# dremovd/PPO

Measured on AMD Instinct MI355X. Metric: env-steps/sec (Pong-shaped synthetic, 256 envs/GPU), higher is better.
Workload: dtype f32

## Files before the change

### ppo_amd/csrc/stack_fused.hip

```cpp
#include <cstdlib>
#include <type_traits>

#include "common.h"
#include "conv_stage.h"
#include "mfma.h"

#ifndef PPO_TAIL_SPLIT
#define PPO_TAIL_SPLIT 2
#endif

namespace ppo {
namespace {

constexpr int kScrPitchS = 20;

struct StackTailArgs {
    const float *in;
    const float *w[4];
    const float *bias[4];
    const float *mask[4];
    float *save[4];
    int n_images;
};

template <int C, int H, int W, int MT, int NW, int NSPLIT>
struct StackCfg {
    static constexpr int ROWS = H + 2;
    static constexpr int G = 4;
    static constexpr int PLANE_RAW = ROWS * W + 2 * G;
    static constexpr int PLANE = PLANE_RAW + ((16 - PLANE_RAW % 32) + 32) % 32;
    static constexpr int NT = C / 16;
    static constexpr int NTL = NT / NSPLIT;
    static constexpr int WAVES = NW * NSPLIT;
    static constexpr int KS = 9 * (C / 4);
    static constexpr int NPIX = H * W;
    static constexpr int MTILES = (NPIX + 15) / 16;
    static constexpr int LDS_MAP = C * PLANE;
    static constexpr size_t LDS_BYTES = (size_t)2 * LDS_MAP * 4;
    static_assert(C % 16 == 0, "channel tiles of 16");
    static_assert(MTILES == MT * NW, "one group of MT pixel tiles per wave");
    static_assert(NT % NSPLIT == 0, "channel tiles split evenly");
};

template <int C, int H, int W, int MT, int NW, int NSPLIT, bool BACKWARD>
__global__ __launch_bounds__(NW * NSPLIT * 64) void stack_tail_kernel(StackTailArgs a)
{
    using S = StackCfg<C, H, W, MT, NW, NSPLIT>;
    constexpr int NT = S::NTL, KS = S::KS, PLANE = S::PLANE, G = S::G;
    extern __shared__ __align__(16) float smem[];
    const int tid = threadIdx.x, lane = tid & 63, l15 = lane & 15, g = lane >> 4;
    const int wave = (tid >> 6) % NW;
    const int n0 = ((tid >> 6) / NW) * NT;

    zero_lds<2 * S::LDS_MAP, S::WAVES * 64>(smem, tid);
    __syncthreads();

    int pix[MT], lofs[MT];
    float hi_l[MT], hi_r[MT];
#pragma unroll
    for (int m = 0; m < MT; ++m) {
        const int p = (wave * MT + m) * 16 + l15;
        pix[m] = p;
        const int pc = p < S::NPIX ? p : 0;
        lofs[m] = G + pc - 1 + g * PLANE;
        hi_l[m] = (pc % W == 0) ? 0.f : INFINITY;
        hi_r[m] = (pc % W == W - 1) ? 0.f : INFINITY;
    }

    float wa[NT][KS];
    auto load_weights = [&](int layer) {
        const float4 *pw = reinterpret_cast<const float4 *>(a.w[layer]);
#pragma unroll
        for (int s4 = 0; s4 < KS / 4; ++s4)
#pragma unroll
            for (int n = 0; n < NT; ++n) {
                const float4 v = pw[(s4 * S::NT + n0 + n) * 64 + lane];
                wa[n][4 * s4 + 0] = v.x;
                wa[n][4 * s4 + 1] = v.y;
                wa[n][4 * s4 + 2] = v.z;
                wa[n][4 * s4 + 3] = v.w;
            }
    };
    load_weights(0);

    for (int img = blockIdx.x; img < a.n_images; img += gridDim.x) {
        __syncthreads();
        stage_band_chunk_dma<C, H, W, S::ROWS, PLANE, G, S::WAVES>(a.in, img, 0, smem, tid);
        const size_t img_off = (size_t)img * C * H * W;

#pragma unroll 1
        for (int layer = 0; layer < 4; ++layer) {
            float bias_r[NT][4];
#pragma unroll
            for (int n = 0; n < NT; ++n)
#pragma unroll
                for (int r = 0; r < 4; ++r) bias_r[n][r] = BACKWARD ? 0.f : a.bias[layer][(n0 + n) * 16 + g * 4 + r];
            float gate[BACKWARD ? MT : 1][NT][4];
            if constexpr (BACKWARD) {
                const __amdgpu_buffer_rsrc_t mask = buffer_of(a.mask[layer] + img_off);
#pragma unroll
                for (int m = 0; m < MT; ++m)
#pragma unroll
                    for (int n = 0; n < NT; ++n)
#pragma unroll
                        for (int r = 0; r < 4; ++r)
                            gate[m][n][r] = buffer_f32(mask, pix[m] < S::NPIX ? (((n0 + n) * 16 + g * 4 + r) * (H * W) + pix[m]) * 4
                                                                              : kOutside);
            }

            __syncthreads();
            const int odd = layer & 1;
            const int src = odd ? S::LDS_MAP : 0;
            int base[MT];
#pragma unroll
            for (int m = 0; m < MT; ++m) base[m] = lofs[m] + src;

            f32x4 acc[NT][MT];
#pragma unroll
            for (int n = 0; n < NT; ++n)
#pragma unroll
                for (int m = 0; m < MT; ++m) acc[n][m] = f32x4{0.f, 0.f, 0.f, 0.f};

            constexpr int SB = (MT * NT >= 4) ? 2 : 4;
            constexpr int NB = (KS + SB - 1) / SB;
            float raw[2][SB][MT];
            auto load_block = [&](int j, float (&r)[SB][MT]) {
#pragma unroll
                for (int u = 0; u < SB; ++u) {
                    const int s = j * SB + u;
                    if (s < KS) {
                        const int tap = s / (C / 4), cs = s % (C / 4);
                        const int tap_off = (tap / 3) * W + (tap % 3);
#pragma unroll
                        for (int m = 0; m < MT; ++m) r[u][m] = smem[base[m] + cs * 4 * PLANE + tap_off];
                    }
                }
            };
            load_block(0, raw[0]);
#pragma unroll
            for (int j = 0; j < NB; ++j) {
                float bv[SB][MT];
#pragma unroll
                for (int u = 0; u < SB; ++u) {
                    const int s = j * SB + u;
                    if (s < KS) {
                        const int kx = (s / (C / 4)) % 3;
#pragma unroll
                        for (int m = 0; m < MT; ++m) {
                            float x = raw[j & 1][u][m];
                            if (kx != 1) {
                                const float hi = kx == 0 ? hi_l[m] : hi_r[m];
                                x = __builtin_amdgcn_fmed3f(x, BACKWARD ? -hi : 0.f, hi);
                            } else if (!BACKWARD) {
                                x = relu1(x);
                            }
                            bv[u][m] = x;
                        }
                    }
                }
                __builtin_amdgcn_sched_barrier(0);
                if (j + 1 < NB) load_block(j + 1, raw[(j + 1) & 1]);
#pragma unroll
                for (int u = 0; u < SB; ++u) {
                    const int s = j * SB + u;
                    if (s < KS) {
#pragma unroll
                        for (int m = 0; m < MT; ++m)
#pragma unroll
                            for (int n = 0; n < NT; ++n) acc[n][m] = mfma16(wa[n][s], bv[u][m], acc[n][m]);
                    }
                }
                __builtin_amdgcn_sched_barrier(0);
            }

            __builtin_amdgcn_sched_barrier(0);
            load_weights((layer + 1) & 3);
            float *dst = smem + (odd ? 0 : S::LDS_MAP);
            float *save = a.save[layer];
            __builtin_amdgcn_sched_barrier(0);
            float skip[MT][NT][4];
#pragma unroll
            for (int m = 0; m < MT; ++m)
#pragma unroll
                for (int n = 0; n < NT; ++n)
#pragma unroll
                    for (int r = 0; r < 4; ++r)
                        skip[m][n][r] = odd ? smem[((n0 + n) * 16 + g * 4 + r) * PLANE + G + W + (pix[m] < S::NPIX ? pix[m] : 0)] : 0.f;
#pragma unroll
            for (int m = 0; m < MT; ++m) {
                if (pix[m] < S::NPIX) {
#pragma unroll
                    for (int n = 0; n < NT; ++n)
#pragma unroll
                        for (int r = 0; r < 4; ++r) {
                            const int co = (n0 + n) * 16 + g * 4 + r;
                            const int lo = co * PLANE + G + W + pix[m];
                            float val = acc[n][m][r] + bias_r[n][r];
                            if constexpr (BACKWARD) val = gate[m][n][r] > 0.f ? val : 0.f;
                            if (odd) val = val + skip[m][n][r];
                            dst[lo] = val;
                            if (save) save[img_off + (size_t)co * (H * W) + pix[m]] = val;
                        }
                }
            }
        }
    }
}

template <int C, int H, int W, int MT, int NW, int NSPLIT, bool BACKWARD>
int launch_stack_tail(const StackTailArgs &args, hipStream_t st)
{
    using S = StackCfg<C, H, W, MT, NW, NSPLIT>;
    auto kern = stack_tail_kernel<C, H, W, MT, NW, NSPLIT, BACKWARD>;
    static int wg_per_cu = 0;
    if (wg_per_cu == 0) {
        hipError_t e = hipFuncSetAttribute(reinterpret_cast<const void *>(kern), hipFuncAttributeMaxDynamicSharedMemorySize,
                                           (int)S::LDS_BYTES);
        if (e != hipSuccess) return fail(PPO_E_HIP, "stack_tail: hipFuncSetAttribute: %s", hipGetErrorString(e));
        int nb = 0;
        e = hipOccupancyMaxActiveBlocksPerMultiprocessor(&nb, kern, S::WAVES * 64, S::LDS_BYTES);
        if (e != hipSuccess) return fail(PPO_E_HIP, "stack_tail: occupancy query: %s", hipGetErrorString(e));
        wg_per_cu = nb < 1 ? 1 : nb;
    }
    int grid = 256 * wg_per_cu;
    if (grid > args.n_images) grid = args.n_images;
    hipLaunchKernelGGL(kern, dim3(grid), dim3(S::WAVES * 64), S::LDS_BYTES, st, args);
    return check_launch("stack_tail_kernel");
}

template <int C, int H, int W, int TR>
struct ShiftCfg {
    static_assert(C == 16, "one channel tile per wave");
    static constexpr int NW = 16;
    static constexpr int GW = 8;
    static constexpr int G = 4;
    static constexpr int ROWS = H + 6;
    static constexpr int PLANE_RAW = ROWS * W + 2 * G;
    static constexpr int PLANE = PLANE_RAW + ((16 - PLANE_RAW % 32) + 32) % 32;
    static constexpr int KS = 9 * (C / 4);
    static constexpr int NBANDS = (H + TR - 1) / TR;
    static constexpr int NPIX = TR * W;
    static constexpr int MTILES = (NPIX + 15) / 16;
    static constexpr int MT = MTILES / GW;
    static constexpr int LDS_MAP = C * PLANE;
    static constexpr int SCR = MT * 16 * kScrPitchS;
    static constexpr size_t LDS_BYTES = (size_t)(LDS_MAP + GW * SCR) * 4;
    static_assert(H % TR == 0 && MTILES == MT * GW, "whole bands, tiles split evenly over a group's waves");
    static_assert((H * W) % 4 == 0 && NPIX % 4 == 0 && W % 2 == 0, "float4 epilogue on whole quads");
    static_assert(LDS_BYTES <= 160 * 1024, "map + scratch must fit the CU's LDS");
};

template <int C, int H, int W, int TR, bool BACKWARD>
__global__ __launch_bounds__(1024) void stack_shift_kernel(StackTailArgs a)
{
    using S = ShiftCfg<C, H, W, TR>;
    constexpr int KS = S::KS, PLANE = S::PLANE, G = S::G, MT = S::MT, NW = S::NW;
    extern __shared__ __align__(16) float smem[];
    const int tid = threadIdx.x, lane = tid & 63, l15 = lane & 15, g = lane >> 4, wave = tid >> 6;
    const int grp = __builtin_amdgcn_readfirstlane(wave / S::GW), wv = wave % S::GW;
    const int ch = lane >> 2, quad = lane & 3;
    float *scr = smem + S::LDS_MAP + wv * S::SCR;

    int lofs[MT], p4[MT];
    float hi_l[MT], hi_r[MT];
#pragma unroll
    for (int m = 0; m < MT; ++m) {
        const int p = (wv * MT + m) * 16 + l15;
        lofs[m] = G + p - 1 + g * PLANE;
        hi_l[m] = (p % W == 0) ? 0.f : INFINITY;
        hi_r[m] = (p % W == W - 1) ? 0.f : INFINITY;
        p4[m] = (wv * MT + m) * 16 + quad * 4;
    }

    for (int img = blockIdx.x; img < a.n_images; img += gridDim.x) {
        const size_t img_off = (size_t)img * C * H * W;
        __syncthreads();
        for (int i = tid; i < C * 6 * W; i += NW * 64) {
            const int c = i / (6 * W), r = (i / W) % 6, x = i % W;
            smem[c * PLANE + G + (r < 5 ? r : H + 5) * W + x] = 0.f;
        }
        for (int i = tid; i < C * 2 * G; i += NW * 64)
            smem[(i / (2 * G)) * PLANE + ((i % (2 * G)) < G ? (i % G) : G + S::ROWS * W + (i % G))] = 0.f;
        {
            using gptr_t = const __attribute__((address_space(1))) void *;
            using lptr_t = __attribute__((address_space(3))) void *;
            constexpr int N4 = H * W / 4, REQ = (N4 + 63) / 64;
            const int w0 = __builtin_amdgcn_readfirstlane(wave);
            for (int c = w0; c < C; c += NW) {
                const float *g0 = a.in + img_off + (size_t)c * H * W;
                float *l0 = smem + c * PLANE + G + 5 * W;
#pragma unroll
                for (int q = 0; q < REQ; ++q)
                    if (q * 64 + lane < N4)
                        __builtin_amdgcn_global_load_lds((gptr_t)(g0 + (q * 64 + lane) * 4), (lptr_t)(l0 + q * 256), 16, 0, 0);
            }
        }

#pragma unroll 1
        for (int layer = 0; layer < 4; ++layer) {
            float wa[KS];
            const float4 *pw = reinterpret_cast<const float4 *>(a.w[layer]);
#pragma unroll
            for (int s4 = 0; s4 < KS / 4; ++s4) {
                const float4 v = pw[s4 * 64 + lane];
                wa[4 * s4 + 0] = v.x, wa[4 * s4 + 1] = v.y, wa[4 * s4 + 2] = v.z, wa[4 * s4 + 3] = v.w;
            }
            const float bias_c = BACKWARD ? 0.f : a.bias[layer][ch];
            const int odd = layer & 1;
            const float *res = odd ? (layer == 1 ? a.in : a.save[1]) + img_off : nullptr;
            const float *mask = BACKWARD ? a.mask[layer] + img_off : nullptr;
            float *save = a.save[layer] ? a.save[layer] + img_off : nullptr;
            const __amdgpu_buffer_rsrc_t mask_b = buffer_of(mask, mask != nullptr), res_b = buffer_of(res, res != nullptr);
            const int in_row = 5 - layer;

            f32x4 acc[MT];
            float4 gate4[MT], res4[MT];

            __syncthreads();
#pragma unroll 1
            for (int hs = 0; hs <= S::NBANDS; ++hs) {
                if ((hs & 1) == grp) {
                    if (hs < S::NBANDS) {
                        const int y0 = hs * TR;
                        const int chan_off = ch * (H * W) + y0 * W;
#pragma unroll
                        for (int m = 0; m < MT; ++m) {
                            const bool live = p4[m] < S::NPIX;
                            const int off = live ? (chan_off + p4[m]) * 4 : kOutside;
                            if constexpr (BACKWARD) gate4[m] = buffer_f32x4(mask_b, off);
                            res4[m] = buffer_f32x4(res_b, off);
                        }
                        int base[MT];
#pragma unroll
                        for (int m = 0; m < MT; ++m) {
                            base[m] = lofs[m] + (y0 - 1 + in_row) * W;
                            acc[m] = f32x4{0.f, 0.f, 0.f, 0.f};
                        }
                        constexpr int SB = 2;
                        constexpr int NB = (KS + SB - 1) / SB;
                        float raw[2][SB][MT];
                        auto load_block = [&](int j, float (&r)[SB][MT]) {
#pragma unroll
                            for (int u = 0; u < SB; ++u) {
                                const int s = j * SB + u;
                                if (s < KS) {
                                    const int tap = s / (C / 4), cs = s % (C / 4);
                                    const int tap_off = (tap / 3) * W + (tap % 3);
#pragma unroll
                                    for (int m = 0; m < MT; ++m) r[u][m] = smem[base[m] + cs * 4 * PLANE + tap_off];
                                }
                            }
                        };
                        load_block(0, raw[0]);
#pragma unroll
                        for (int j = 0; j < NB; ++j) {
                            float bv[SB][MT];
#pragma unroll
                            for (int u = 0; u < SB; ++u) {
                                const int s = j * SB + u;
                                if (s < KS) {
                                    const int kx = (s / (C / 4)) % 3;
#pragma unroll
                                    for (int m = 0; m < MT; ++m) {
                                        float x = raw[j & 1][u][m];
                                        if (kx != 1) {
                                            const float hi = kx == 0 ? hi_l[m] : hi_r[m];
                                            x = __builtin_amdgcn_fmed3f(x, BACKWARD ? -hi : 0.f, hi);
                                        } else if (!BACKWARD) {
                                            x = relu1(x);
                                        }
                                        bv[u][m] = x;
                                    }
                                }
                            }
                            __builtin_amdgcn_sched_barrier(0);
                            if (j + 1 < NB) load_block(j + 1, raw[(j + 1) & 1]);
#pragma unroll
                            for (int u = 0; u < SB; ++u) {
                                const int s = j * SB + u;
                                if (s < KS) {
#pragma unroll
                                    for (int m = 0; m < MT; ++m) acc[m] = mfma16(wa[s], bv[u][m], acc[m]);
                                }
                            }
                            __builtin_amdgcn_sched_barrier(0);
                        }
                    } else if (layer < 3) {
                        for (int i = tid % (S::GW * 64); i < C * W; i += S::GW * 64)
                            smem[(i / W) * PLANE + G + (H + in_row - 1) * W + i % W] = 0.f;
                    }
                } else if (hs >= 1) {
                    const int y0 = (hs - 1) * TR;
                    const int chan_off = ch * (H * W) + y0 * W;
#pragma unroll
                    for (int m = 0; m < MT; ++m)
#pragma unroll
                        for (int r = 0; r < 4; ++r) scr[(m * 16 + g * 4 + r) * kScrPitchS + l15] = acc[m][r];
                    __builtin_amdgcn_wave_barrier();
                    float *out_row = smem + ch * PLANE + G + (y0 + in_row - 1) * W;
#pragma unroll
                    for (int m = 0; m < MT; ++m) {
                        if (p4[m] >= S::NPIX) continue;
                        const float4 o = *reinterpret_cast<const float4 *>(scr + (m * 16 + ch) * kScrPitchS + quad * 4);
                        const float ov[4] = {o.x, o.y, o.z, o.w};
                        const float gv[4] = {gate4[m].x, gate4[m].y, gate4[m].z, gate4[m].w};
                        const float rv[4] = {res4[m].x, res4[m].y, res4[m].z, res4[m].w};
                        float v[4];
#pragma unroll
                        for (int e = 0; e < 4; ++e) {
                            float val = ov[e] + bias_c;
                            if constexpr (BACKWARD) val = gv[e] > 0.f ? val : 0.f;
                            v[e] = val + rv[e];
                        }
                        if (layer < 3) {
                            *reinterpret_cast<float2 *>(out_row + p4[m]) = make_float2(v[0], v[1]);
                            *reinterpret_cast<float2 *>(out_row + p4[m] + 2) = make_float2(v[2], v[3]);
                        }
                        if (save) *reinterpret_cast<float4 *>(save + chan_off + p4[m]) = make_float4(v[0], v[1], v[2], v[3]);
                    }
                    __builtin_amdgcn_wave_barrier();
                }
                __syncthreads();
            }
        }
    }
}

template <int C, int H, int W, int TR, bool BACKWARD>
int launch_stack_shift(const StackTailArgs &args, hipStream_t st)
{
    using S = ShiftCfg<C, H, W, TR>;
    auto kern = stack_shift_kernel<C, H, W, TR, BACKWARD>;
    static bool attr_set = false;
    if (!attr_set) {
        hipError_t e = hipFuncSetAttribute(reinterpret_cast<const void *>(kern), hipFuncAttributeMaxDynamicSharedMemorySize,
                                           (int)S::LDS_BYTES);
        if (e != hipSuccess) return fail(PPO_E_HIP, "stack_shift: hipFuncSetAttribute: %s", hipGetErrorString(e));
        attr_set = true;
    }
    int grid = 256;
    if (grid > args.n_images) grid = args.n_images;
    hipLaunchKernelGGL(kern, dim3(grid), dim3(S::NW * 64), S::LDS_BYTES, st, args);
    return check_launch("stack_shift_kernel");
}

template <int I, int N, class F>
__device__ __forceinline__ void static_for(F &&f)
{
    if constexpr (I < N) {
        f(std::integral_constant<int, I>{});
        static_for<I + 1, N>(f);
    }
}

struct LaneMap {
    template <int MT>
    struct T {
        int pix[MT], lofs[MT];
        float hi_l[MT], hi_r[MT];
    };
};

template <int H, int W, int PLANE, int G, int MT>
__device__ __forceinline__ void lane_map_init(LaneMap::T<MT> &lm, int pixel_wave, int l15, int g)
{
#pragma unroll
    for (int m = 0; m < MT; ++m) {
        const int p = (pixel_wave * MT + m) * 16 + l15;
        lm.pix[m] = p;
        const int pc = p < H * W ? p : 0;
        lm.lofs[m] = G + pc - 1 + g * PLANE;
        lm.hi_l[m] = (pc % W == 0) ? 0.f : INFINITY;
        lm.hi_r[m] = (pc % W == W - 1) ? 0.f : INFINITY;
    }
}

template <int C, int H, int W, int MT, int NTOT, int NT, bool RELU_IN, bool GATED = false>
__device__ __forceinline__ void resident_conv(float *smem, int src_off, int dst_off, bool residual, const float *wpk,
                                              const float *bias, float *save, const LaneMap::T<MT> &lm, int n0, int lane,
                                              const float *mask = nullptr)
{
    constexpr int ROWS = H + 2, G = 4, PLANE_RAW = ROWS * W + 2 * G;
    constexpr int PLANE = PLANE_RAW + ((16 - PLANE_RAW % 32) + 32) % 32;
    constexpr int KS = 9 * (C / 4);
    const int g = lane >> 4;
    float wa[NT][KS];
    const float4 *pw = reinterpret_cast<const float4 *>(wpk);
#pragma unroll
    for (int s4 = 0; s4 < KS / 4; ++s4)
#pragma unroll
        for (int n = 0; n < NT; ++n) {
            const float4 v = pw[(s4 * NTOT + n0 + n) * 64 + lane];
            wa[n][4 * s4 + 0] = v.x;
            wa[n][4 * s4 + 1] = v.y;
            wa[n][4 * s4 + 2] = v.z;
            wa[n][4 * s4 + 3] = v.w;
        }
    float bias_r[NT][4];
#pragma unroll
    for (int n = 0; n < NT; ++n)
#pragma unroll
        for (int r = 0; r < 4; ++r) bias_r[n][r] = (GATED || !bias) ? 0.f : bias[(n0 + n) * 16 + g * 4 + r];
    float gate[GATED ? MT : 1][NT][4];
    if constexpr (GATED) {
        const __amdgpu_buffer_rsrc_t mask_b = buffer_of(mask);
#pragma unroll
        for (int m = 0; m < MT; ++m)
#pragma unroll
            for (int n = 0; n < NT; ++n)
#pragma unroll
                for (int r = 0; r < 4; ++r)
                    gate[m][n][r] = buffer_f32(mask_b, lm.pix[m] < H * W ? (((n0 + n) * 16 + g * 4 + r) * (H * W) + lm.pix[m]) * 4
                                                                         : kOutside);
    }

    __syncthreads();
    int base[MT];
#pragma unroll
    for (int m = 0; m < MT; ++m) base[m] = lm.lofs[m] + src_off;
    f32x4 acc[NT][MT];
#pragma unroll
    for (int n = 0; n < NT; ++n)
#pragma unroll
        for (int m = 0; m < MT; ++m) acc[n][m] = f32x4{0.f, 0.f, 0.f, 0.f};

    constexpr int SB = (MT * NT >= 4) ? 2 : 4;
    constexpr int NB = (KS + SB - 1) / SB;
    float raw[2][SB][MT];
    auto load_block = [&](int j, float (&r)[SB][MT]) {
#pragma unroll
        for (int u = 0; u < SB; ++u) {
            const int s = j * SB + u;
            if (s < KS) {
                const int tap = s / (C / 4), cs = s % (C / 4);
                const int tap_off = (tap / 3) * W + (tap % 3);
#pragma unroll
                for (int m = 0; m < MT; ++m) r[u][m] = smem[base[m] + cs * 4 * PLANE + tap_off];
            }
        }
    };
    load_block(0, raw[0]);
    static_for<0, NB>([&](auto jc) {
        constexpr int j = decltype(jc)::value;
        float bv[SB][MT];
#pragma unroll
        for (int u = 0; u < SB; ++u) {
            const int s = j * SB + u;
            if (s < KS) {
                const int kx = (s / (C / 4)) % 3;
#pragma unroll
                for (int m = 0; m < MT; ++m) {
                    float x = raw[j & 1][u][m];
                    if (kx != 1) {
                        const float hi = kx == 0 ? lm.hi_l[m] : lm.hi_r[m];
                        x = __builtin_amdgcn_fmed3f(x, RELU_IN ? 0.f : -hi, hi);
                    } else if (RELU_IN) {
                        x = relu1(x);
                    }
                    bv[u][m] = x;
                }
            }
        }
        __builtin_amdgcn_sched_barrier(0);
        if constexpr (j + 1 < NB) load_block(j + 1, raw[(j + 1) & 1]);
#pragma unroll
        for (int u = 0; u < SB; ++u) {
            const int s = j * SB + u;
            if (s < KS) {
#pragma unroll
                for (int m = 0; m < MT; ++m)
#pragma unroll
                    for (int n = 0; n < NT; ++n) acc[n][m] = mfma16(wa[n][s], bv[u][m], acc[n][m]);
            }
        }
        __builtin_amdgcn_sched_barrier(0);
    });
#pragma unroll
    for (int m = 0; m < MT; ++m) {
        if (lm.pix[m] < H * W) {
#pragma unroll
            for (int n = 0; n < NT; ++n)
#pragma unroll
                for (int r = 0; r < 4; ++r) {
                    const int co = (n0 + n) * 16 + g * 4 + r;
                    const int lo = dst_off + co * PLANE + G + W + lm.pix[m];
                    float val = acc[n][m][r] + bias_r[n][r];
                    if constexpr (GATED) val = gate[m][n][r] > 0.f ? val : 0.f;
                    if (residual) val = val + smem[lo];
                    smem[lo] = val;
                    if (save) save[(size_t)co * (H * W) + lm.pix[m]] = val;
                }
        }
    }
}

struct StackFullArgs {
    const float *in;
    const float *w[5];
    const float *bias[5];
    float *pooled;
    uint8_t *argmax;
    float *save[4];
    const float *pre_w[4];
    const float *pre_bias[4];
    float *pre_save[4];
    int has_pre;
    int n_images;
};

template <int C, int HI, int WI, int MTI, int HO, int WO, int MTO, int NW, int NSPLIT>
__global__ __launch_bounds__(NW * NSPLIT * 64) void stack_full_kernel(StackFullArgs a)
{
    using SI = StackCfg<C, HI, WI, MTI, NW, NSPLIT>;
    using SO = StackCfg<C, HO, WO, MTO, NW, NSPLIT>;
    static_assert(HO == (HI + 1) / 2 && WO == (WI + 1) / 2, "3x3 / stride 2 / pad 1 pooling");
    static_assert(2 * SO::LDS_MAP <= SI::LDS_MAP, "the small maps reuse the input map's LDS");
    constexpr int NT = SI::NTL, WAVES = SI::WAVES, THREADS = WAVES * 64;
    constexpr int A_OFF = 0, B_OFF = SI::LDS_MAP, X_OFF = 0, Y_OFF = SO::LDS_MAP;
    extern __shared__ __align__(16) float smem[];
    const int tid = threadIdx.x, lane = tid & 63, l15 = lane & 15, g = lane >> 4;
    const int wave = tid >> 6, pixel_wave = wave % NW, n0 = (wave / NW) * NT;

    LaneMap::T<MTI> lmi;
    LaneMap::T<MTO> lmo;
    lane_map_init<HI, WI, SI::PLANE, SI::G, MTI>(lmi, pixel_wave, l15, g);
    lane_map_init<HO, WO, SO::PLANE, SO::G, MTO>(lmo, pixel_wave, l15, g);

    if (a.has_pre) zero_lds<SI::LDS_MAP, THREADS>(smem + B_OFF, tid);

    for (int img = blockIdx.x; img < a.n_images; img += gridDim.x) {
        __syncthreads();
        zero_lds<SI::LDS_MAP, THREADS>(smem + A_OFF, tid);
        __syncthreads();
        stage_band_chunk_dma<C, HI, WI, SI::ROWS, SI::PLANE, SI::G, WAVES>(a.in, img, 0, smem + A_OFF, tid);
        if (a.has_pre) {
            const size_t big_img = (size_t)img * C * HI * WI;
#pragma unroll 1
            for (int layer = 0; layer < 4; ++layer) {
                const int odd = layer & 1;
                float *save = a.pre_save[layer] ? a.pre_save[layer] + big_img : nullptr;
                resident_conv<C, HI, WI, MTI, SI::NT, NT, true>(smem, odd ? B_OFF : A_OFF, odd ? A_OFF : B_OFF, odd != 0,
                                                                a.pre_w[layer], a.pre_bias[layer], save, lmi, n0, lane);
            }
        }
        resident_conv<C, HI, WI, MTI, SI::NT, NT, false>(smem, A_OFF, B_OFF, false, a.w[0], a.bias[0], nullptr, lmi, n0, lane);
        __syncthreads();
        zero_lds<2 * SO::LDS_MAP, THREADS>(smem + X_OFF, tid);
        __syncthreads();
        {
            constexpr int RPW = 64 / WO;
            const int sub = lane / WO, xo = lane % WO;
            const size_t out_img = (size_t)img * C * HO * WO;
            for (int u0 = wave * RPW; u0 < C * HO; u0 += WAVES * RPW) {
                const int u = u0 + sub;
                const int co = u / HO, yo = u % HO;
                if (sub < RPW && co < C) {
                    const float *src = smem + B_OFF + co * SI::PLANE + SI::G + WI + (2 * yo - 1) * WI + 2 * xo - 1;
                    float best;
                    int best_tap;
                    pool_window_lds<HI % 2 == 0, WI % 2 == 0>(src, WI, yo > 0, 2 * yo + 1 < HI, xo > 0, 2 * xo + 1 < WI, best, best_tap);
                    smem[X_OFF + co * SO::PLANE + SO::G + WO + yo * WO + xo] = best;
                    const size_t oi = out_img + ((size_t)co * HO + yo) * WO + xo;
                    if (a.pooled) a.pooled[oi] = best;
                    if (a.argmax) a.argmax[oi] = (uint8_t)best_tap;
                }
            }
        }
        const size_t out_img = (size_t)img * C * HO * WO;
#pragma unroll 1
        for (int layer = 0; layer < 4; ++layer) {
            const int odd = layer & 1;
            float *save = a.save[layer] ? a.save[layer] + out_img : nullptr;
            resident_conv<C, HO, WO, MTO, SO::NT, NT, true>(smem, odd ? Y_OFF : X_OFF, odd ? X_OFF : Y_OFF, odd != 0,
                                                            a.w[1 + layer], a.bias[1 + layer], save, lmo, n0, lane);
        }
    }
}

struct StackFullBwdArgs {
    const float *g;
    const float *w[5];
    const float *mask[4];
    const uint8_t *argmax;
    float *save[4];
    float *dc;
    float *g_prev;
    int n_images;
};

template <int C, int HI, int WI, int MTI, int HO, int WO, int MTO, int NW, int NSPLIT>
__global__ __launch_bounds__(NW * NSPLIT * 64) void stack_full_bwd_kernel(StackFullBwdArgs a)
{
    using SI = StackCfg<C, HI, WI, MTI, NW, NSPLIT>;
    using SO = StackCfg<C, HO, WO, MTO, NW, NSPLIT>;
    static_assert(2 * SO::LDS_MAP <= SI::LDS_MAP, "the small maps live inside the first big map's LDS");
    constexpr int NT = SI::NTL, WAVES = SI::WAVES, THREADS = WAVES * 64;
    constexpr int A_OFF = 0, B_OFF = SI::LDS_MAP, X_OFF = 0, Y_OFF = SO::LDS_MAP;
    extern __shared__ __align__(16) float smem[];
    const int tid = threadIdx.x, lane = tid & 63, l15 = lane & 15, g = lane >> 4;
    const int wave = tid >> 6, pixel_wave = wave % NW, n0 = (wave / NW) * NT;

    LaneMap::T<MTI> lmi;
    LaneMap::T<MTO> lmo;
    lane_map_init<HI, WI, SI::PLANE, SI::G, MTI>(lmi, pixel_wave, l15, g);
    lane_map_init<HO, WO, SO::PLANE, SO::G, MTO>(lmo, pixel_wave, l15, g);

    zero_lds<SI::LDS_MAP, THREADS>(smem + B_OFF, tid);

    for (int img = blockIdx.x; img < a.n_images; img += gridDim.x) {
        __syncthreads();
        zero_lds<2 * SO::LDS_MAP, THREADS>(smem + X_OFF, tid);
        __syncthreads();
        stage_band_chunk_dma<C, HO, WO, SO::ROWS, SO::PLANE, SO::G, WAVES>(a.g, img, 0, smem + X_OFF, tid);
        const size_t small_img = (size_t)img * C * HO * WO, big_img = (size_t)img * C * HI * WI;
#pragma unroll 1
        for (int layer = 0; layer < 4; ++layer) {
            const int odd = layer & 1;
            resident_conv<C, HO, WO, MTO, SO::NT, NT, false, true>(smem, odd ? Y_OFF : X_OFF, odd ? X_OFF : Y_OFF, odd != 0,
                                                                   a.w[layer], nullptr, a.save[layer] + small_img, lmo, n0,
                                                                   lane, a.mask[layer] + small_img);
        }
        __syncthreads();
        {
            const uint8_t *am = a.argmax + small_img;
            for (int e = tid; e < C * HI * WI; e += THREADS) {
                const int co = e / (HI * WI), r = e % (HI * WI);
                const int iy = r / WI, ix = r % WI;
                const int k = ix >> 1, oy0 = iy >> 1;
                const int ky0 = (iy & 1) ? 2 : 1;
                const bool has_oy1 = (iy & 1) && (oy0 + 1 < HO);
                const bool odd_x = ix & 1;
                const bool has_ox1 = odd_x && (k + 1 < WO);
                const int kx0 = odd_x ? 2 : 1;
                const float *gx = smem + X_OFF + co * SO::PLANE + SO::G + WO;
                const uint8_t *ac = am + co * (HO * WO);
                float sum = 0.f;
                {
                    const int i00 = oy0 * WO + k;
                    if (ac[i00] == ky0 * 3 + kx0) sum += gx[i00];
                    if (has_ox1 && ac[i00 + 1] == ky0 * 3 + 0) sum += gx[i00 + 1];
                }
                if (has_oy1) {
                    const int i10 = (oy0 + 1) * WO + k;
                    if (ac[i10] == kx0) sum += gx[i10];
                    if (has_ox1 && ac[i10 + 1] == 0) sum += gx[i10 + 1];
                }
                smem[B_OFF + co * SI::PLANE + SI::G + WI + r] = sum;
                a.dc[big_img + e] = sum;
            }
        }
        resident_conv<C, HI, WI, MTI, SI::NT, NT, false, false>(smem, B_OFF, A_OFF, false, a.w[4], nullptr,
                                                                a.g_prev + big_img, lmi, n0, lane);
    }
}

template <int C, int HI, int WI, int MTI, int HO, int WO, int MTO, int NW, int NSPLIT>
int launch_stack_full_bwd(const StackFullBwdArgs &args, hipStream_t st)
{
    using SI = StackCfg<C, HI, WI, MTI, NW, NSPLIT>;
    constexpr size_t kLds = 2 * (size_t)SI::LDS_MAP * 4;
    auto kern = stack_full_bwd_kernel<C, HI, WI, MTI, HO, WO, MTO, NW, NSPLIT>;
    static bool ready = false;
    if (!ready) {
        hipError_t e = hipFuncSetAttribute(reinterpret_cast<const void *>(kern), hipFuncAttributeMaxDynamicSharedMemorySize,
                                           (int)kLds);
        if (e != hipSuccess) return fail(PPO_E_HIP, "stack_full_bwd: hipFuncSetAttribute: %s", hipGetErrorString(e));
        ready = true;
    }
    const int grid = args.n_images < 256 ? args.n_images : 256;
    hipLaunchKernelGGL(kern, dim3(grid), dim3(SI::WAVES * 64), kLds, st, args);
    return check_launch("stack_full_bwd_kernel");
}

template <int C, int HI, int WI, int MTI, int HO, int WO, int MTO, int NW, int NSPLIT>
int launch_stack_full(const StackFullArgs &args, hipStream_t st)
{
    using SI = StackCfg<C, HI, WI, MTI, NW, NSPLIT>;
    constexpr size_t kLds = 2 * (size_t)SI::LDS_MAP * 4;
    auto kern = stack_full_kernel<C, HI, WI, MTI, HO, WO, MTO, NW, NSPLIT>;
    static bool ready = false;
    if (!ready) {
        hipError_t e = hipFuncSetAttribute(reinterpret_cast<const void *>(kern), hipFuncAttributeMaxDynamicSharedMemorySize,
                                           (int)kLds);
        if (e != hipSuccess) return fail(PPO_E_HIP, "stack_full: hipFuncSetAttribute: %s", hipGetErrorString(e));
        ready = true;
    }
    const int grid = args.n_images < 256 ? args.n_images : 256;
    hipLaunchKernelGGL(kern, dim3(grid), dim3(SI::WAVES * 64), kLds, st, args);
    return check_launch("stack_full_kernel");
}


struct ChainSplitArgs {
    const float *in;
    const float *pre_w[4];
    const float *pre_bias[4];
    const float *w[5];
    const float *bias[5];
    float *out;
    float *xbuf;
    uint32_t *flags;
    uint32_t *ctl;
    int n_images;
    int skip;
};

constexpr int kSplitWaves = 8;
constexpr uint32_t kSpinLimit = 1u << 21;

template <int C, int HI, int WI, int HO, int WO>
__global__ __launch_bounds__(kSplitWaves * 64) void stack_chain_split_kernel(ChainSplitArgs a)
{
    static_assert(C == 32, "two channel tiles: one per workgroup of a pair");
    using SI = StackCfg<C, HI, WI, 7, 4, 2>;
    using SO = StackCfg<C, HO, WO, 2, 4, 2>;
    constexpr int MTI = 4, MTO = 2, WAVES = kSplitWaves, THREADS = WAVES * 64;
    static_assert(SI::MTILES <= MTI * WAVES && SO::MTILES == MTO * 4 && WAVES == 8, "every pixel tile has a wave");
    static_assert(2 * SO::LDS_MAP <= SI::LDS_MAP, "the small maps reuse the input map's LDS");
    constexpr int A_OFF = 0, B_OFF = SI::LDS_MAP, X_OFF = 0, Y_OFF = SO::LDS_MAP;
    extern __shared__ __align__(16) float smem[];
    const int tid = threadIdx.x, lane = tid & 63, l15 = lane & 15, g = lane >> 4;
    const int wave = tid >> 6;
    const int b = blockIdx.x;
    const int h = (b >> 3) & 1;
    const int pair0 = (b & 7) | ((b >> 4) << 3);
    const int n_pairs = (gridDim.x >> 4) << 3;

    LaneMap::T<MTI> lmi;
    LaneMap::T<MTO> lmo;
    lane_map_init<HI, WI, SI::PLANE, SI::G, MTI>(lmi, wave, l15, g);
    lane_map_init<HO, WO, SO::PLANE, SO::G, MTO>(lmo, wave & 3, l15, g);

    const uint32_t base = __hip_atomic_load(a.ctl, __ATOMIC_RELAXED, __HIP_MEMORY_SCOPE_AGENT) * 8u;
    const uint32_t fault = __hip_atomic_load(a.ctl + 3, __ATOMIC_RELAXED, __HIP_MEMORY_SCOPE_AGENT);
    const uint32_t spin_limit = fault ? 1u << 10 : kSpinLimit;
    bool gave_up = false;
    zero_lds<SI::LDS_MAP, THREADS>(smem + B_OFF, tid);

    for (int img = pair0; img < a.n_images; img += n_pairs) {
        uint32_t *flag_own = a.flags + 2 * img + h, *flag_other = a.flags + 2 * img + (1 - h);
        float *slots = a.xbuf + (size_t)img * 2 * C * HI * WI;
        uint32_t step = 0;
        auto exchange = [&](int dst_off, float *slot, bool fetch) {
            ++step;
            asm volatile("s_waitcnt vmcnt(0)" ::: "memory");
            __syncthreads();
            if (tid == 0) {
                if (!(fault && h == 1))
                    __hip_atomic_store(flag_own, base + step, __ATOMIC_RELAXED, __HIP_MEMORY_SCOPE_AGENT);
                uint32_t it = 0;
                while (!(a.skip & 1) && !gave_up &&
                       __hip_atomic_load(flag_other, __ATOMIC_RELAXED, __HIP_MEMORY_SCOPE_AGENT) < base + step) {
                    if (++it > spin_limit ||
                        ((it & 1023u) == 0 && __hip_atomic_load(a.ctl + 2, __ATOMIC_RELAXED, __HIP_MEMORY_SCOPE_AGENT))) {
                        __hip_atomic_store(a.ctl + 2, 1u, __ATOMIC_RELAXED, __HIP_MEMORY_SCOPE_AGENT);
                        gave_up = true;
                        break;
                    }
                    __builtin_amdgcn_s_sleep(2);
                }
            }
            __syncthreads();
            if (fetch)
                stage_band_chunk_dma<16, HI, WI, SI::ROWS, SI::PLANE, SI::G, WAVES, 16>(slot + (size_t)(1 - h) * 16 * HI * WI, 0, 0,
                                                                                       smem + dst_off + (1 - h) * 16 * SI::PLANE, tid);
        };

        __syncthreads();
        zero_lds<SI::LDS_MAP, THREADS>(smem + A_OFF, tid);
        __syncthreads();
        stage_band_chunk_dma<C, HI, WI, SI::ROWS, SI::PLANE, SI::G, WAVES>(a.in, img, 0, smem + A_OFF, tid);
#pragma unroll 1
        for (int layer = 0; layer < 4; ++layer) {
            const int odd = layer & 1;
            float *slot = slots + (size_t)(layer & 1) * C * HI * WI;
            resident_conv<C, HI, WI, MTI, 2, 1, true>(smem, odd ? B_OFF : A_OFF, odd ? A_OFF : B_OFF, odd != 0, a.pre_w[layer],
                                                      a.pre_bias[layer], slot, lmi, h, lane);
            exchange(odd ? A_OFF : B_OFF, slot, true);
        }
        resident_conv<C, HI, WI, MTI, 2, 1, false>(smem, A_OFF, B_OFF, false, a.w[0], a.bias[0], slots, lmi, h, lane);
        exchange(B_OFF, slots, h == 0);
        if (h != 0 || (a.skip & 2)) continue;
        __syncthreads();
        zero_lds<2 * SO::LDS_MAP, THREADS>(smem + X_OFF, tid);
        __syncthreads();
        {
            constexpr int RPW = 64 / WO;
            const int sub = lane / WO, xo = lane % WO;
            for (int u0 = wave * RPW; u0 < C * HO; u0 += WAVES * RPW) {
                const int u = u0 + sub;
                const int co = u / HO, yo = u % HO;
                if (sub < RPW && co < C) {
                    const float *src = smem + B_OFF + co * SI::PLANE + SI::G + WI + (2 * yo - 1) * WI + 2 * xo - 1;
                    float best;
                    int best_tap;
                    pool_window_lds<HI % 2 == 0, WI % 2 == 0>(src, WI, yo > 0, 2 * yo + 1 < HI, xo > 0, 2 * xo + 1 < WI, best, best_tap);
                    smem[X_OFF + co * SO::PLANE + SO::G + WO + yo * WO + xo] = best;
                }
            }
        }
        float *out_img = a.out + (size_t)img * C * HO * WO;
#pragma unroll 1
        for (int layer = 0; layer < 4; ++layer) {
            const int odd = layer & 1;
            resident_conv<C, HO, WO, MTO, 2, 1, true>(smem, odd ? Y_OFF : X_OFF, odd ? X_OFF : Y_OFF, odd != 0, a.w[1 + layer],
                                                      a.bias[1 + layer], layer == 3 ? out_img : nullptr, lmo, wave >> 2, lane);
        }
    }
    __syncthreads();
    if (tid == 0) {
        const uint32_t done = __hip_atomic_fetch_add(a.ctl + 1, 1u, __ATOMIC_RELAXED, __HIP_MEMORY_SCOPE_AGENT);
        if (done == gridDim.x - 1) {
            __hip_atomic_store(a.ctl + 1, 0u, __ATOMIC_RELAXED, __HIP_MEMORY_SCOPE_AGENT);
            __hip_atomic_fetch_add(a.ctl, 1u, __ATOMIC_RELAXED, __HIP_MEMORY_SCOPE_AGENT);
        }
    }
}

template <int C, int HI, int WI, int HO, int WO>
int launch_chain_split(const ChainSplitArgs &args, hipStream_t st)
{
    using SI = StackCfg<C, HI, WI, 7, 4, 2>;
    constexpr size_t kLds = 2 * (size_t)SI::LDS_MAP * 4;
    auto kern = stack_chain_split_kernel<C, HI, WI, HO, WO>;
    static bool ready = false;
    if (!ready) {
        hipError_t e = hipFuncSetAttribute(reinterpret_cast<const void *>(kern), hipFuncAttributeMaxDynamicSharedMemorySize,
                                           (int)kLds);
        if (e != hipSuccess) return fail(PPO_E_HIP, "stack_chain_split: hipFuncSetAttribute: %s", hipGetErrorString(e));
        ready = true;
    }
    int groups = (args.n_images + 7) / 8;
    if (groups > 16) groups = 16;
    hipLaunchKernelGGL(kern, dim3(16 * groups), dim3(kSplitWaves * 64), kLds, st, args);
    return check_launch("stack_chain_split_kernel");
}

}
}

extern "C" int ppo_impala_stack_tail_supported(int channels, int h, int w)
{
    if (channels == 16) return (h == 42 && w == 42) || (h == 32 && w == 32);
    return channels == 32 && ((h == 11 && w == 11) || (h == 21 && w == 21) || (h == 16 && w == 16) || (h == 8 && w == 8));
}

extern "C" int ppo_impala_stack_tail_forward_f32(const float *in, const float *const *packed_weights,
                                                 const float *const *biases, float *a0, float *q0, float *a1, float *q1,
                                                 int n_images, int channels, int h, int w, void *stream)
{
    using namespace ppo;
    if (n_images < 0) return fail(PPO_E_INVALID, "ppo_impala_stack_tail_forward_f32: negative batch");
    if (n_images == 0) return PPO_OK;
    if (!in || !packed_weights || !biases || !q1)
        return fail(PPO_E_INVALID, "ppo_impala_stack_tail_forward_f32: null pointer");
    StackTailArgs args;
    args.in = in;
    for (int l = 0; l < 4; ++l) {
        if (!packed_weights[l] || !biases[l])
            return fail(PPO_E_INVALID, "ppo_impala_stack_tail_forward_f32: null weights / bias of layer %d", l);
        if (!aligned(packed_weights[l], 16))
            return fail(PPO_E_ALIGN, "ppo_impala_stack_tail_forward_f32: packed weights must be 16-byte aligned");
        args.w[l] = packed_weights[l];
        args.bias[l] = biases[l];
        args.mask[l] = nullptr;
    }
    if (!aligned(in, 4)) return fail(PPO_E_ALIGN, "ppo_impala_stack_tail_forward_f32: input must be 4-byte aligned");
    args.save[0] = a0;
    args.save[1] = q0;
    args.save[2] = a1;
    args.save[3] = q1;
    args.n_images = n_images;
    hipStream_t st = as_stream(stream);
    if (channels == 16) {
        if (!q0) return fail(PPO_E_INVALID, "ppo_impala_stack_tail_forward_f32: the 16-channel form needs q0 (its second block re-reads it)");
        if (!aligned(in, 16) || !aligned(q0, 16) || !aligned(q1, 16) || (a0 && !aligned(a0, 16)) || (a1 && !aligned(a1, 16)))
            return fail(PPO_E_ALIGN, "ppo_impala_stack_tail_forward_f32: the 16-channel form needs 16-byte aligned maps");
        if (h == 42 && w == 42) return launch_stack_shift<16, 42, 42, 6, false>(args, st);
        if (h == 32 && w == 32) return launch_stack_shift<16, 32, 32, 8, false>(args, st);
    }
    if (channels == 32 && h == 11 && w == 11) return launch_stack_tail<32, 11, 11, 2, 4, PPO_TAIL_SPLIT, false>(args, st);
    if (channels == 32 && h == 21 && w == 21) return launch_stack_tail<32, 21, 21, 7, 4, PPO_TAIL_SPLIT, false>(args, st);
    if (channels == 32 && h == 16 && w == 16) return launch_stack_tail<32, 16, 16, 4, 4, PPO_TAIL_SPLIT, false>(args, st);
    if (channels == 32 && h == 8 && w == 8) return launch_stack_tail<32, 8, 8, 1, 4, PPO_TAIL_SPLIT, false>(args, st);
    return fail(PPO_E_INVALID, "ppo_impala_stack_tail_forward_f32: no kernel for %d channels at %dx%d", channels, h, w);
}

extern "C" int ppo_impala_stack_tail_backward_f32(const float *g, const float *const *packed_weights_t,
                                                  const float *const *masks, float *da1, float *g1, float *da0, float *g0,
                                                  int n_images, int channels, int h, int w, void *stream)
{
    using namespace ppo;
    if (n_images < 0) return fail(PPO_E_INVALID, "ppo_impala_stack_tail_backward_f32: negative batch");
    if (n_images == 0) return PPO_OK;
    if (!g || !packed_weights_t || !masks || !da1 || !g1 || !da0 || !g0)
        return fail(PPO_E_INVALID, "ppo_impala_stack_tail_backward_f32: null pointer");
    StackTailArgs args;
    args.in = g;
    for (int l = 0; l < 4; ++l) {
        if (!packed_weights_t[l] || !masks[l])
            return fail(PPO_E_INVALID, "ppo_impala_stack_tail_backward_f32: null weights / mask of layer %d", l);
        if (!aligned(packed_weights_t[l], 16))
            return fail(PPO_E_ALIGN, "ppo_impala_stack_tail_backward_f32: packed weights must be 16-byte aligned");
        args.w[l] = packed_weights_t[l];
        args.bias[l] = nullptr;
        args.mask[l] = masks[l];
    }
    args.save[0] = da1;
    args.save[1] = g1;
    args.save[2] = da0;
    args.save[3] = g0;
    args.n_images = n_images;
    hipStream_t st = as_stream(stream);
    if (channels == 16) {
        for (const void *ptr : {(const void *)g, (const void *)da1, (const void *)g1, (const void *)da0, (const void *)g0,
                                (const void *)masks[0], (const void *)masks[1], (const void *)masks[2], (const void *)masks[3]})
            if (!aligned(ptr, 16))
                return fail(PPO_E_ALIGN, "ppo_impala_stack_tail_backward_f32: the 16-channel form needs 16-byte aligned maps");
        if (h == 42 && w == 42) return launch_stack_shift<16, 42, 42, 6, true>(args, st);
        if (h == 32 && w == 32) return launch_stack_shift<16, 32, 32, 8, true>(args, st);
    }
    if (channels == 32 && h == 11 && w == 11) return launch_stack_tail<32, 11, 11, 2, 4, PPO_TAIL_SPLIT, true>(args, st);
    if (channels == 32 && h == 21 && w == 21) return launch_stack_tail<32, 21, 21, 7, 4, PPO_TAIL_SPLIT, true>(args, st);
    if (channels == 32 && h == 16 && w == 16) return launch_stack_tail<32, 16, 16, 4, 4, PPO_TAIL_SPLIT, true>(args, st);
    if (channels == 32 && h == 8 && w == 8) return launch_stack_tail<32, 8, 8, 1, 4, PPO_TAIL_SPLIT, true>(args, st);
    return fail(PPO_E_INVALID, "ppo_impala_stack_tail_backward_f32: no kernel for %d channels at %dx%d", channels, h, w);
}

extern "C" int ppo_impala_stack_full_supported(int channels, int h, int w)
{
    return channels == 32 && ((h == 21 && w == 21) || (h == 16 && w == 16));
}

extern "C" int ppo_impala_stack_full_forward_f32(const float *in, const float *const *packed_weights,
                                                 const float *const *biases, float *pooled, uint8_t *argmax, float *a0,
                                                 float *q0, float *a1, float *q1, int n_images, int channels, int h, int w,
                                                 void *stream)
{
    using namespace ppo;
    if (n_images < 0) return fail(PPO_E_INVALID, "ppo_impala_stack_full_forward_f32: negative batch");
    if (n_images == 0) return PPO_OK;
    if (!in || !packed_weights || !biases || !q1)
        return fail(PPO_E_INVALID, "ppo_impala_stack_full_forward_f32: null pointer");
    StackFullArgs args;
    args.in = in;
    for (int l = 0; l < 5; ++l) {
        if (!packed_weights[l] || !biases[l])
            return fail(PPO_E_INVALID, "ppo_impala_stack_full_forward_f32: null weights / bias of layer %d", l);
        if (!aligned(packed_weights[l], 16))
            return fail(PPO_E_ALIGN, "ppo_impala_stack_full_forward_f32: packed weights must be 16-byte aligned");
        args.w[l] = packed_weights[l];
        args.bias[l] = biases[l];
    }
    args.pooled = pooled;
    args.argmax = argmax;
    args.save[0] = a0;
    args.save[1] = q0;
    args.save[2] = a1;
    args.save[3] = q1;
    args.has_pre = 0;
    for (int l = 0; l < 4; ++l) {
        args.pre_w[l] = nullptr;
        args.pre_bias[l] = nullptr;
        args.pre_save[l] = nullptr;
    }
    args.n_images = n_images;
    if (channels == 32 && h == 21 && w == 21)
        return launch_stack_full<32, 21, 21, 7, 11, 11, 2, 4, 2>(args, as_stream(stream));
    if (channels == 32 && h == 16 && w == 16)
        return launch_stack_full<32, 16, 16, 4, 8, 8, 1, 4, 2>(args, as_stream(stream));
    return fail(PPO_E_INVALID, "ppo_impala_stack_full_forward_f32: no kernel for %d channels at %dx%d", channels, h, w);
}

extern "C" int ppo_impala_stack_chain_forward_f32(const float *in, const float *const *pre_packed_weights,
                                                  const float *const *pre_biases, float *pre_a0, float *pre_q0,
                                                  float *pre_a1, float *pre_q1, const float *const *packed_weights,
                                                  const float *const *biases, float *pooled, uint8_t *argmax, float *a0,
                                                  float *q0, float *a1, float *q1, int n_images, int channels, int h, int w,
                                                  void *stream)
{
    using namespace ppo;
    if (n_images < 0) return fail(PPO_E_INVALID, "ppo_impala_stack_chain_forward_f32: negative batch");
    if (n_images == 0) return PPO_OK;
    if (!in || !pre_packed_weights || !pre_biases || !packed_weights || !biases || !q1)
        return fail(PPO_E_INVALID, "ppo_impala_stack_chain_forward_f32: null pointer");
    StackFullArgs args;
    args.in = in;
    for (int l = 0; l < 5; ++l) {
        if (!packed_weights[l] || !biases[l] || (l < 4 && (!pre_packed_weights[l] || !pre_biases[l])))
            return fail(PPO_E_INVALID, "ppo_impala_stack_chain_forward_f32: null weights / bias of layer %d", l);
        if (!aligned(packed_weights[l], 16) || (l < 4 && !aligned(pre_packed_weights[l], 16)))
            return fail(PPO_E_ALIGN, "ppo_impala_stack_chain_forward_f32: packed weights must be 16-byte aligned");
        args.w[l] = packed_weights[l];
        args.bias[l] = biases[l];
        if (l < 4) {
            args.pre_w[l] = pre_packed_weights[l];
            args.pre_bias[l] = pre_biases[l];
        }
    }
    args.pre_save[0] = pre_a0;
    args.pre_save[1] = pre_q0;
    args.pre_save[2] = pre_a1;
    args.pre_save[3] = pre_q1;
    args.has_pre = 1;
    args.pooled = pooled;
    args.argmax = argmax;
    args.save[0] = a0;
    args.save[1] = q0;
    args.save[2] = a1;
    args.save[3] = q1;
    args.n_images = n_images;
    if (channels == 32 && h == 21 && w == 21)
        return launch_stack_full<32, 21, 21, 7, 11, 11, 2, 4, 2>(args, as_stream(stream));
    if (channels == 32 && h == 16 && w == 16)
        return launch_stack_full<32, 16, 16, 4, 8, 8, 1, 4, 2>(args, as_stream(stream));
    return fail(PPO_E_INVALID, "ppo_impala_stack_chain_forward_f32: no kernel for %d channels at %dx%d", channels, h, w);
}

extern "C" int ppo_impala_stack_full_backward_f32(const float *g, const float *const *packed_weights_t,
                                                  const float *const *masks, const uint8_t *argmax, float *da1, float *g1,
                                                  float *da0, float *g0, float *dc, float *g_prev, int n_images,
                                                  int channels, int h, int w, void *stream)
{
    using namespace ppo;
    if (n_images < 0) return fail(PPO_E_INVALID, "ppo_impala_stack_full_backward_f32: negative batch");
    if (n_images == 0) return PPO_OK;
    if (!g || !packed_weights_t || !masks || !argmax || !da1 || !g1 || !da0 || !g0 || !dc || !g_prev)
        return fail(PPO_E_INVALID, "ppo_impala_stack_full_backward_f32: null pointer");
    StackFullBwdArgs args;
    args.g = g;
    for (int l = 0; l < 5; ++l) {
        if (!packed_weights_t[l] || (l < 4 && !masks[l]))
            return fail(PPO_E_INVALID, "ppo_impala_stack_full_backward_f32: null weights / mask of layer %d", l);
        if (!aligned(packed_weights_t[l], 16))
            return fail(PPO_E_ALIGN, "ppo_impala_stack_full_backward_f32: packed weights must be 16-byte aligned");
        args.w[l] = packed_weights_t[l];
        if (l < 4) args.mask[l] = masks[l];
    }
    args.argmax = argmax;
    args.save[0] = da1;
    args.save[1] = g1;
    args.save[2] = da0;
    args.save[3] = g0;
    args.dc = dc;
    args.g_prev = g_prev;
    args.n_images = n_images;
    if (channels == 32 && h == 21 && w == 21)
        return launch_stack_full_bwd<32, 21, 21, 7, 11, 11, 2, 4, 2>(args, as_stream(stream));
    if (channels == 32 && h == 16 && w == 16)
        return launch_stack_full_bwd<32, 16, 16, 4, 8, 8, 1, 4, 2>(args, as_stream(stream));
    return fail(PPO_E_INVALID, "ppo_impala_stack_full_backward_f32: no kernel for %d channels at %dx%d", channels, h, w);
}

extern "C" size_t ppo_impala_stack_chain_split_workspace_bytes(int n_images, int channels, int h, int w)
{
    const size_t slots = (size_t)n_images * 2 * channels * h * w * sizeof(float);
    const size_t flags = ((size_t)n_images * 2 * sizeof(uint32_t) + 15) & ~(size_t)15;
    return slots + flags + 16;
}

extern "C" int ppo_impala_stack_chain_split_forward_f32(const float *in, const float *const *pre_packed_weights,
                                                        const float *const *pre_biases,
                                                        const float *const *packed_weights, const float *const *biases,
                                                        float *q1, void *workspace, size_t workspace_bytes, int n_images,
                                                        int channels, int h, int w, void *stream)
{
    using namespace ppo;
    if (n_images < 0) return fail(PPO_E_INVALID, "ppo_impala_stack_chain_split_forward_f32: negative batch");
    if (n_images == 0) return PPO_OK;
    if (!in || !pre_packed_weights || !pre_biases || !packed_weights || !biases || !q1 || !workspace)
        return fail(PPO_E_INVALID, "ppo_impala_stack_chain_split_forward_f32: null pointer");
    if (!(channels == 32 && h == 21 && w == 21))
        return fail(PPO_E_INVALID, "ppo_impala_stack_chain_split_forward_f32: no kernel for %d channels at %dx%d", channels, h, w);
    if (workspace_bytes < ppo_impala_stack_chain_split_workspace_bytes(n_images, channels, h, w) || !aligned(workspace, 16))
        return fail(PPO_E_INVALID, "ppo_impala_stack_chain_split_forward_f32: workspace too small or misaligned");
    ChainSplitArgs args;
    args.in = in;
    for (int l = 0; l < 5; ++l) {
        if (!packed_weights[l] || !biases[l] || (l < 4 && (!pre_packed_weights[l] || !pre_biases[l])))
            return fail(PPO_E_INVALID, "ppo_impala_stack_chain_split_forward_f32: null weights / bias of layer %d", l);
        if (!aligned(packed_weights[l], 16) || (l < 4 && !aligned(pre_packed_weights[l], 16)))
            return fail(PPO_E_ALIGN, "ppo_impala_stack_chain_split_forward_f32: packed weights must be 16-byte aligned");
        args.w[l] = packed_weights[l];
        args.bias[l] = biases[l];
        if (l < 4) {
            args.pre_w[l] = pre_packed_weights[l];
            args.pre_bias[l] = pre_biases[l];
        }
    }
    args.out = q1;
    const size_t slots = (size_t)n_images * 2 * channels * h * w * sizeof(float);
    const size_t flags = ((size_t)n_images * 2 * sizeof(uint32_t) + 15) & ~(size_t)15;
    args.xbuf = static_cast<float *>(workspace);
    args.flags = reinterpret_cast<uint32_t *>(static_cast<char *>(workspace) + slots);
    args.ctl = reinterpret_cast<uint32_t *>(static_cast<char *>(workspace) + slots + flags);
    args.n_images = n_images;
#ifdef PPO_TUNE_TIMING_AIDS
    static const int skip = getenv("PPO_AMD_SPLIT_SKIP") ? atoi(getenv("PPO_AMD_SPLIT_SKIP")) : 0;
    args.skip = skip;
#else
    args.skip = 0;
#endif
    return launch_chain_split<32, 21, 21, 11, 11>(args, as_stream(stream));
}
```

Before: 95720.

## Pad LDS rows with zero halo columns and apply relu once at store time

Gives each LDS row a pitch of W+2, so the left and right halo columns are zero padding. This removes the per-tap fmed3 edge masking in the inner MFMA loop. The relu is moved out of the per-tap operand path into the epilogue store and the input staging, so each activation is clamped once instead of nine times. Input staging changes from async global_load_lds to register float2 loads, because the padded pitch no longer matches contiguous global rows. Per-channel-group base offsets are precomputed. The costs are a larger LDS footprint per plane and a synchronous staging path.

```diff
diff --git a/ppo_amd/csrc/stack_fused.hip b/ppo_amd/csrc/stack_fused.hip
--- a/ppo_amd/csrc/stack_fused.hip
+++ b/ppo_amd/csrc/stack_fused.hip
@@ -235,7 +235,8 @@
     static constexpr int GW = 8;
     static constexpr int G = 4;
     static constexpr int ROWS = H + 6;
-    static constexpr int PLANE_RAW = ROWS * W + 2 * G;
+    static constexpr int RP = W + 2;
+    static constexpr int PLANE_RAW = ROWS * RP + 2 * G;
     static constexpr int PLANE = PLANE_RAW + ((16 - PLANE_RAW % 32) + 32) % 32;
     static constexpr int KS = 9 * (C / 4);
     static constexpr int NBANDS = (H + TR - 1) / TR;
@@ -246,7 +247,8 @@
     static constexpr int SCR = MT * 16 * kScrPitchS;
     static constexpr size_t LDS_BYTES = (size_t)(LDS_MAP + GW * SCR) * 4;
     static_assert(H % TR == 0 && MTILES == MT * GW, "whole bands, tiles split evenly over a group's waves");
-    static_assert((H * W) % 4 == 0 && NPIX % 4 == 0 && W % 2 == 0, "float4 epilogue on whole quads");
+    static_assert((H * W) % 4 == 0 && NPIX % 4 == 0 && W % 2 == 0, "float4 epilogue on whole quads, float2 LDS stores");
+    static_assert(RP % 2 == 0 && PLANE % 2 == 0 && G % 2 == 0, "8-byte aligned pixel pairs in LDS");
     static_assert(LDS_BYTES <= 160 * 1024, "map + scratch must fit the CU's LDS");
 };
 
@@ -254,45 +256,47 @@
 __global__ __launch_bounds__(1024) void stack_shift_kernel(StackTailArgs a)
 {
     using S = ShiftCfg<C, H, W, TR>;
-    constexpr int KS = S::KS, PLANE = S::PLANE, G = S::G, MT = S::MT, NW = S::NW;
+    constexpr int KS = S::KS, PLANE = S::PLANE, G = S::G, MT = S::MT, NW = S::NW, RP = S::RP;
     extern __shared__ __align__(16) float smem[];
     const int tid = threadIdx.x, lane = tid & 63, l15 = lane & 15, g = lane >> 4, wave = tid >> 6;
     const int grp = __builtin_amdgcn_readfirstlane(wave / S::GW), wv = wave % S::GW;
     const int ch = lane >> 2, quad = lane & 3;
     float *scr = smem + S::LDS_MAP + wv * S::SCR;
 
-    int lofs[MT], p4[MT];
-    float hi_l[MT], hi_r[MT];
+    int lofs[MT], p4[MT], o4[MT];
 #pragma unroll
     for (int m = 0; m < MT; ++m) {
         const int p = (wv * MT + m) * 16 + l15;
-        lofs[m] = G + p - 1 + g * PLANE;
-        hi_l[m] = (p % W == 0) ? 0.f : INFINITY;
-        hi_r[m] = (p % W == W - 1) ? 0.f : INFINITY;
+        lofs[m] = G + (p / W) * RP + p % W - 1 + g * PLANE;
         p4[m] = (wv * MT + m) * 16 + quad * 4;
-    }
-
+        o4[m] = (p4[m] / W) * RP + p4[m] % W;
+    }
+
+    zero_lds<S::LDS_MAP, NW * 64>(smem, tid);
     for (int img = blockIdx.x; img < a.n_images; img += gridDim.x) {
         const size_t img_off = (size_t)img * C * H * W;
         __syncthreads();
-        for (int i = tid; i < C * 6 * W; i += NW * 64) {
-            const int c = i / (6 * W), r = (i / W) % 6, x = i % W;
-            smem[c * PLANE + G + (r < 5 ? r : H + 5) * W + x] = 0.f;
-        }
-        for (int i = tid; i < C * 2 * G; i += NW * 64)
-            smem[(i / (2 * G)) * PLANE + ((i % (2 * G)) < G ? (i % G) : G + S::ROWS * W + (i % G))] = 0.f;
+        for (int i = tid; i < C * 6 * RP; i += NW * 64) {
+            const int c = i / (6 * RP), r = (i / RP) % 6, x = i % RP;
+            smem[c * PLANE + G + (r < 5 ? r : H + 5) * RP + x] = 0.f;
+        }
         {
-            using gptr_t = const __attribute__((address_space(1))) void *;
-            using lptr_t = __attribute__((address_space(3))) void *;
-            constexpr int N4 = H * W / 4, REQ = (N4 + 63) / 64;
-            const int w0 = __builtin_amdgcn_readfirstlane(wave);
-            for (int c = w0; c < C; c += NW) {
-                const float *g0 = a.in + img_off + (size_t)c * H * W;
-                float *l0 = smem + c * PLANE + G + 5 * W;
-#pragma unroll
-                for (int q = 0; q < REQ; ++q)
-                    if (q * 64 + lane < N4)
-                        __builtin_amdgcn_global_load_lds((gptr_t)(g0 + (q * 64 + lane) * 4), (lptr_t)(l0 + q * 256), 16, 0, 0);
+            constexpr int W2 = W / 2, RPI = 64 / W2, NI = H / RPI;
+            static_assert(H % RPI == 0, "whole rows per staging instruction");
+            const int x2 = lane % W2, yl = lane / W2;
+            for (int c = __builtin_amdgcn_readfirstlane(wave); c < C; c += NW) {
+                if (yl < RPI) {
+                    const float2 *g0 = reinterpret_cast<const float2 *>(a.in + img_off + (size_t)c * H * W + yl * W) + x2;
+                    float2 *l0 = reinterpret_cast<float2 *>(smem + c * PLANE + G + (5 + yl) * RP + 2 * x2);
+                    float2 v[NI];
+#pragma unroll
+                    for (int k = 0; k < NI; ++k) v[k] = g0[k * RPI * W2];
+#pragma unroll
+                    for (int k = 0; k < NI; ++k) {
+                        if constexpr (!BACKWARD) v[k] = make_float2(relu1(v[k].x), relu1(v[k].y));
+                        l0[k * RPI * (RP / 2)] = v[k];
+                    }
+                }
             }
         }
 
@@ -330,10 +334,12 @@
                             if constexpr (BACKWARD) gate4[m] = buffer_f32x4(mask_b, off);
                             res4[m] = buffer_f32x4(res_b, off);
                         }
-                        int base[MT];
+                        constexpr int NCG = C / 4;
+                        int base[NCG][MT];
 #pragma unroll
                         for (int m = 0; m < MT; ++m) {
-                            base[m] = lofs[m] + (y0 - 1 + in_row) * W;
+#pragma unroll
+                            for (int cg = 0; cg < NCG; ++cg) base[cg][m] = (lofs[m] + (y0 - 1 + in_row) * RP + cg * 4 * PLANE) & 0xffff;
                             acc[m] = f32x4{0.f, 0.f, 0.f, 0.f};
                         }
                         constexpr int SB = 2;
@@ -345,49 +351,30 @@
                                 const int s = j * SB + u;
                                 if (s < KS) {
                                     const int tap = s / (C / 4), cs = s % (C / 4);
-                                    const int tap_off = (tap / 3) * W + (tap % 3);
-#pragma unroll
-                                    for (int m = 0; m < MT; ++m) r[u][m] = smem[base[m] + cs * 4 * PLANE + tap_off];
+                                    const int tap_off = (tap / 3) * RP + (tap % 3);
+#pragma unroll
+                                    for (int m = 0; m < MT; ++m) r[u][m] = smem[base[cs][m] + tap_off];
                                 }
                             }
                         };
                         load_block(0, raw[0]);
 #pragma unroll
                         for (int j = 0; j < NB; ++j) {
-                            float bv[SB][MT];
+                            __builtin_amdgcn_sched_barrier(0);
+                            if (j + 1 < NB) load_block(j + 1, raw[(j + 1) & 1]);
 #pragma unroll
                             for (int u = 0; u < SB; ++u) {
                                 const int s = j * SB + u;
                                 if (s < KS) {
-                                    const int kx = (s / (C / 4)) % 3;
-#pragma unroll
-                                    for (int m = 0; m < MT; ++m) {
-                                        float x = raw[j & 1][u][m];
-                                        if (kx != 1) {
-                                            const float hi = kx == 0 ? hi_l[m] : hi_r[m];
-                                            x = __builtin_amdgcn_fmed3f(x, BACKWARD ? -hi : 0.f, hi);
-                                        } else if (!BACKWARD) {
-                                            x = relu1(x);
-                                        }
-                                        bv[u][m] = x;
-                                    }
-                                }
-                            }
-                            __builtin_amdgcn_sched_barrier(0);
-                            if (j + 1 < NB) load_block(j + 1, raw[(j + 1) & 1]);
-#pragma unroll
-                            for (int u = 0; u < SB; ++u) {
-                                const int s = j * SB + u;
-                                if (s < KS) {
-#pragma unroll
-                                    for (int m = 0; m < MT; ++m) acc[m] = mfma16(wa[s], bv[u][m], acc[m]);
+#pragma unroll
+                                    for (int m = 0; m < MT; ++m) acc[m] = mfma16(wa[s], raw[j & 1][u][m], acc[m]);
                                 }
                             }
                             __builtin_amdgcn_sched_barrier(0);
                         }
                     } else if (layer < 3) {
                         for (int i = tid % (S::GW * 64); i < C * W; i += S::GW * 64)
-                            smem[(i / W) * PLANE + G + (H + in_row - 1) * W + i % W] = 0.f;
+                            smem[(i / W) * PLANE + G + (H + in_row - 1) * RP + i % W] = 0.f;
                     }
                 } else if (hs >= 1) {
                     const int y0 = (hs - 1) * TR;
@@ -397,7 +384,7 @@
 #pragma unroll
                         for (int r = 0; r < 4; ++r) scr[(m * 16 + g * 4 + r) * kScrPitchS + l15] = acc[m][r];
                     __builtin_amdgcn_wave_barrier();
-                    float *out_row = smem + ch * PLANE + G + (y0 + in_row - 1) * W;
+                    float *out_row = smem + ch * PLANE + G + (y0 + in_row - 1) * RP;
 #pragma unroll
                     for (int m = 0; m < MT; ++m) {
                         if (p4[m] >= S::NPIX) continue;
@@ -413,8 +400,12 @@
                             v[e] = val + rv[e];
                         }
                         if (layer < 3) {
-                            *reinterpret_cast<float2 *>(out_row + p4[m]) = make_float2(v[0], v[1]);
-                            *reinterpret_cast<float2 *>(out_row + p4[m] + 2) = make_float2(v[2], v[3]);
+                            float r4[4];
+#pragma unroll
+                            for (int e = 0; e < 4; ++e) r4[e] = BACKWARD ? v[e] : relu1(v[e]);
+                            const int o2 = ((p4[m] + 2) / W) * RP + (p4[m] + 2) % W;
+                            *reinterpret_cast<float2 *>(out_row + o4[m]) = make_float2(r4[0], r4[1]);
+                            *reinterpret_cast<float2 *>(out_row + o2) = make_float2(r4[2], r4[3]);
                         }
                         if (save) *reinterpret_cast<float4 *>(save + chan_off + p4[m]) = make_float4(v[0], v[1], v[2], v[3]);
                     }
```

After: 97800 (median of 6 runs). 1.02x the previous value.
